# deeppowers/deeppowers

Hardware: AMD Instinct MI355X
Metric: ciphertext-mul/s (N=4096, 4 RNS limbs) (higher is better)
Workload: dtype u64

## Files before the change

deeppowers_amd/csrc/dpfhe_cabi.hip:

```cpp
#include <dlfcn.h>
#include <hip/hip_runtime.h>

#include <algorithm>
#include <atomic>
#include <cstdio>
#include <cstdlib>
#include <cstring>
#include <mutex>
#include <new>
#include <string>
#include <type_traits>
#include <vector>

#include "../../include/dpfhe.h"
#include "base_ext.h"
#include "compact.h"
#include "encode.h"
#include "expand.h"
#include "noise.h"
#include "plain_add.h"
#include "kernels_large.h"
#include "kernels_misc.h"
#include "launch.h"
#include "ntt_core.h"
// ... 1184 lines not shown
}

extern "C" int dpfhe_rescale_bsgs(dpfhe_ctx* c, uint64_t* d_out2, const uint64_t* d_in_qp, const uint64_t* d_addends, size_t n_add, size_t batch, void* stream) {
    const char* what = "dpfhe_rescale_bsgs";
    if (!c) return fail(DPFHE_INVALID_ARGUMENT, what, "null context");
    if (c->n_limbs < 2) return fail(DPFHE_INVALID_STATE, what, "no limb left to drop");
    if (batch == 0) return DPFHE_SUCCESS;
    if (!d_out2 || !d_in_qp || (n_add && !d_addends) || misaligned(d_out2) || misaligned(d_in_qp) || misaligned(d_addends))
        return fail(DPFHE_INVALID_ARGUMENT, what, "null or misaligned buffer");
    const size_t L = c->n_limbs, Ld = L - 1;
    const int n = 1 << c->log2n;
    const int chunks = (n + 511) / 512;
    if (overlaps(d_out2, batch * 2 * Ld * n, d_in_qp, batch * 2 * L * n) || (n_add && overlaps(d_out2, batch * 2 * Ld * n, d_addends, n_add * batch * 2 * Ld * n)))
        return fail(DPFHE_INVALID_ARGUMENT, what, "output overlaps an input");
    const size_t blocks = batch * 2 * Ld * (size_t)chunks;
    if (blocks > kMaxGrid) return fail(DPFHE_INVALID_ARGUMENT, what, "batch too large for one launch");
    DPFHE_ON_DEVICE(c, what);
    hipStream_t s = static_cast<hipStream_t>(stream);
    with_ctx_arith(c, [&](auto arith) {
        hipLaunchKernelGGL((rescale_bsgs_kernel<decltype(arith)>), dim3((unsigned)blocks), dim3(256), 0, s, d_out2, d_in_qp, d_addends, n_add, batch, c->lc, c->d_rescale, (int)L, n, chunks);
    });
    return check_launch("rescale_bsgs kernel launch");
}

extern "C" int dpfhe_apply_galois(dpfhe_ctx* c, uint64_t* d_out, const uint64_t* d_in, size_t n_rns_polys, uint32_t galois_elt, void* stream) {
    if (!c) return fail(DPFHE_INVALID_ARGUMENT, "dpfhe_apply_galois", "null context");
    const unsigned two_n = 2u << c->log2n;
    if (!(galois_elt & 1u) || galois_elt >= two_n) return fail(DPFHE_INVALID_ARGUMENT, "dpfhe_apply_galois", "galois_elt must be odd and < 2N");
    if (n_rns_polys == 0) return DPFHE_SUCCESS;
    if (!d_out || !d_in || misaligned(d_out) || misaligned(d_in) ||
        overlaps(d_out, n_rns_polys * ((size_t)c->n_limbs << c->log2n), d_in, n_rns_polys * ((size_t)c->n_limbs << c->log2n)))
        return fail(DPFHE_INVALID_ARGUMENT, "dpfhe_apply_galois", "null, misaligned or aliased buffer");
    const size_t npolys = n_rns_polys * c->n_limbs;
    if (npolys > kMaxGrid) return fail(DPFHE_INVALID_ARGUMENT, "dpfhe_apply_galois", "batch too large for one launch");
    DPFHE_ON_DEVICE(c, "dpfhe_apply_galois");
    const unsigned inv = galois_inverse(galois_elt, two_n);
    hipLaunchKernelGGL(galois_kernel, dim3((unsigned)npolys), dim3(256), 0, static_cast<hipStream_t>(stream), d_out, d_in, c->lc, (int)c->n_limbs,
                       1 << c->log2n, inv);
    return check_launch("galois kernel launch");
}

extern "C" int dpfhe_matvec_plain(dpfhe_ctx* c, uint64_t* d_y, const uint64_t* d_W, const uint64_t* d_x, size_t rows, size_t cols,
                                  void* stream) {
    if (!c) return fail(DPFHE_INVALID_ARGUMENT, "dpfhe_matvec_plain", "null context");
    if (rows == 0) return DPFHE_SUCCESS;
    if (cols == 0) return fail(DPFHE_INVALID_ARGUMENT, "dpfhe_matvec_plain", "cols must be > 0");
    if (!d_y || !d_W || !d_x || misaligned(d_y) || misaligned(d_W) || misaligned(d_x))
        return fail(DPFHE_INVALID_ARGUMENT, "dpfhe_matvec_plain", "null or misaligned buffer");
    const int n = 1 << c->log2n;
    constexpr int RT = 4;
    DPFHE_ON_DEVICE(c, "dpfhe_matvec_plain");
    hipStream_t s = static_cast<hipStream_t>(stream);
    if (c->fold) {
        constexpr int WPT = kMatvecWpt2;
        const int chunks = (n + 256 * WPT - 1) / (256 * WPT);
        const size_t slabs = c->n_limbs * (size_t)chunks, rtiles = (rows + RT - 1) / RT;
        const size_t blocks = ((slabs + 7) / 8) * 8 * rtiles;
        if (blocks > kMaxGrid) return fail(DPFHE_INVALID_ARGUMENT, "dpfhe_matvec_plain", "too many rows for one launch");
        const bool ntw = rows * cols * ((size_t)c->n_limbs << c->log2n) * sizeof(u64) > ((size_t)256 << 20);
        if (ntw) hipLaunchKernelGGL((matvec_fold_kernel<RT, 2, WPT, true>), dim3((unsigned)blocks), dim3(256), 0, s, d_y, d_W, d_x, c->lc, (int)c->n_limbs, n, chunks, rows,
                                    cols, (size_t)2, 1u, (unsigned)(rtiles * slabs));
        else hipLaunchKernelGGL((matvec_fold_kernel<RT, 2, WPT>), dim3((unsigned)blocks), dim3(256), 0, s, d_y, d_W, d_x, c->lc, (int)c->n_limbs, n, chunks, rows, cols,
                                (size_t)2, 1u, (unsigned)(rtiles * slabs));
        return check_launch("matvec kernel launch");
    }
    const int chunks = (n + 511) / 512;
    const size_t slabs = c->n_limbs * (size_t)chunks;
    const size_t blocks = ((slabs + 7) / 8) * 8 * ((rows + RT - 1) / RT);
    if (blocks > kMaxGrid) return fail(DPFHE_INVALID_ARGUMENT, "dpfhe_matvec_plain", "too many rows for one launch");
    hipLaunchKernelGGL((matvec_kernel<ShoupArith, RT>), dim3((unsigned)blocks), dim3(256), 0, s, d_y, d_W, d_x, c->lc, (int)c->n_limbs, n, chunks, rows, cols);
    return check_launch("matvec kernel launch");
}

template <bool FOLD, int RT, int C, int WPT = 2>
static int matvec_multi_launch(const dpfhe_ctx* c, const char* what, u64* ys, const u64* d_W, const u64* xs, size_t rows, size_t cols, size_t n_rhs, size_t groups,
                               hipStream_t s) {
    const int n = 1 << c->log2n, chunks = (n + 256 * WPT - 1) / (256 * WPT);
    const size_t slabs = c->n_limbs * (size_t)chunks, rtiles = (rows + RT - 1) / RT, tiles = rtiles * slabs;
    const size_t blocks = ((slabs + 7) / 8) * 8 * rtiles * groups;
    if (blocks > kMaxGrid) return fail(DPFHE_INVALID_ARGUMENT, what, "too many rows for one launch");
    if constexpr (!FOLD)
        hipLaunchKernelGGL((matvec_multi_kernel<ShoupArith, RT, C>), dim3((unsigned)blocks), dim3(256), 0, s, ys, d_W, xs, c->lc, (int)c->n_limbs, n, chunks, rows, cols,
                           n_rhs * 2, (unsigned)groups, (unsigned)tiles);
    else if (rows % RT == 0 && cols % FoldArith::kDot30Period == 0)
        hipLaunchKernelGGL((matvec_fold_kernel<RT, C, WPT, false, kMatvecWd, true>), dim3((unsigned)blocks), dim3(256), 0, s, ys, d_W, xs, c->lc, (int)c->n_limbs, n, chunks,
                           rows, cols, n_rhs * 2, (unsigned)groups, (unsigned)tiles);
    else
        hipLaunchKernelGGL((matvec_fold_kernel<RT, C, WPT, false, kMatvecWd>), dim3((unsigned)blocks), dim3(256), 0, s, ys, d_W, xs, c->lc, (int)c->n_limbs, n, chunks,
                           rows, cols, n_rhs * 2, (unsigned)groups, (unsigned)tiles);
    return check_launch("matvec_multi kernel launch");
}

extern "C" int dpfhe_matvec_plain_multi(dpfhe_ctx* c, uint64_t* d_y, const uint64_t* d_W, const uint64_t* d_x, size_t rows, size_t cols, size_t n_rhs,
                                        void* stream) {
    const char* what = "dpfhe_matvec_plain_multi";
    if (!c) return fail(DPFHE_INVALID_ARGUMENT, what, "null context");
    if (rows == 0 || n_rhs == 0) return DPFHE_SUCCESS;
    if (cols == 0) return fail(DPFHE_INVALID_ARGUMENT, what, "cols must be > 0");
    if (!d_y || !d_W || !d_x || misaligned(d_y) || misaligned(d_W) || misaligned(d_x)) return fail(DPFHE_INVALID_ARGUMENT, what, "null or misaligned buffer");
    if (n_rhs == 1) return dpfhe_matvec_plain(c, d_y, d_W, d_x, rows, cols, stream);
    const size_t poly = (size_t)c->n_limbs << c->log2n;
    hipStream_t s = static_cast<hipStream_t>(stream);
    DPFHE_ON_DEVICE(c, what);
    const size_t pairs = n_rhs / 2;
    const uint64_t* x_last = d_x + (n_rhs - 1) * 2 * poly;
    uint64_t* y_last = d_y + (n_rhs - 1) * 2 * poly;
    int rc = DPFHE_SUCCESS;
    if (c->fold) {
        if (pairs) rc = matvec_multi_launch<true, kMatvecRt4, 4, kMatvecWpt4>(c, what, d_y, d_W, d_x, rows, cols, n_rhs, pairs, s);
        if (!rc && (n_rhs & 1)) rc = matvec_multi_launch<true, 4, 2, kMatvecWpt2>(c, what, y_last, d_W, x_last, rows, cols, n_rhs, 1, s);
    } else {
        if (pairs) rc = matvec_multi_launch<false, 4, 4>(c, what, d_y, d_W, d_x, rows, cols, n_rhs, pairs, s);
        if (!rc && (n_rhs & 1)) rc = matvec_multi_launch<false, 4, 2>(c, what, y_last, d_W, x_last, rows, cols, n_rhs, 1, s);
    }
    return rc;
}

extern "C" int dpfhe_matvec_scalar(dpfhe_ctx* c, uint64_t* d_y, const uint64_t* d_w, const uint64_t* d_x, size_t rows, size_t cols,
                                   void* stream) {
    if (!c) return fail(DPFHE_INVALID_ARGUMENT, "dpfhe_matvec_scalar", "null context");
    if (rows == 0) return DPFHE_SUCCESS;
    if (cols == 0) return fail(DPFHE_INVALID_ARGUMENT, "dpfhe_matvec_scalar", "cols must be > 0");
    if (!d_y || !d_w || !d_x || misaligned(d_y) || misaligned(d_x) || (reinterpret_cast<uintptr_t>(d_w) & 7))
        return fail(DPFHE_INVALID_ARGUMENT, "dpfhe_matvec_scalar", "null or misaligned buffer");
    const int n = 1 << c->log2n;
    const int chunks = (n + 511) / 512;
    constexpr int RT = 8;
    const size_t blocks = ((rows + RT - 1) / RT) * c->n_limbs * (size_t)chunks;
    if (blocks > kMaxGrid) return fail(DPFHE_INVALID_ARGUMENT, "dpfhe_matvec_scalar", "too many rows for one launch");
    DPFHE_ON_DEVICE(c, "dpfhe_matvec_scalar");
    hipStream_t s = static_cast<hipStream_t>(stream);
    with_ctx_arith(c, [&](auto arith) {
        hipLaunchKernelGGL((matvec_scalar_kernel<decltype(arith), RT>), dim3((unsigned)blocks), dim3(256), 0, s, d_y, d_w, d_x, c->lc, (int)c->n_limbs, n, chunks, rows, cols);
    });
    return check_launch("matvec_scalar kernel launch");
}

extern "C" int dpfhe_reduce_sum(dpfhe_ctx* c, uint64_t* d_out, const uint64_t* d_in, size_t count, size_t components, void* stream) {
    if (!c) return fail(DPFHE_INVALID_ARGUMENT, "dpfhe_reduce_sum", "null context");
    if (components == 0 || count == 0) return fail(DPFHE_INVALID_ARGUMENT, "dpfhe_reduce_sum", "count and components must be > 0");
    if (!d_out || !d_in || misaligned(d_out) || misaligned(d_in)) return fail(DPFHE_INVALID_ARGUMENT, "dpfhe_reduce_sum", "null or misaligned buffer");
    const size_t blocks = components * c->n_limbs;
    if (blocks > kMaxGrid) return fail(DPFHE_INVALID_ARGUMENT, "dpfhe_reduce_sum", "too many components");
    DPFHE_ON_DEVICE(c, "dpfhe_reduce_sum");
    const int n = 1 << c->log2n;
    const int chunks = (n + 511) / 512;
    const size_t words_per_item = components * c->n_limbs * (size_t)n;
    const size_t want = count / 8 ? count / 8 : 1;
    const unsigned splits = (unsigned)(want < (size_t)kReduceSplits ? want : (size_t)kReduceSplits);
    hipStream_t s = static_cast<hipStream_t>(stream);
    if (blocks * (size_t)chunks * splits > kMaxGrid) return fail(DPFHE_INVALID_ARGUMENT, "dpfhe_reduce_sum", "too many components for one launch");
    HIP_TRY(hipMemsetAsync(d_out, 0, words_per_item * sizeof(u64), s));
    const unsigned poly_chunks = (unsigned)(blocks * chunks);
    unsigned grid = poly_chunks * splits;
    if (count > 512 && grid > 2u * (unsigned)c->n_cu) grid = 2u * (unsigned)c->n_cu;
    hipLaunchKernelGGL(reduce_partial_kernel, dim3(grid), dim3(256), 0, s, d_out, d_in, c->lc, (int)c->n_limbs, n, chunks, count, words_per_item,
                       poly_chunks, splits);
    if (int e = check_launch("reduce_sum partial kernel launch")) return e;
    hipLaunchKernelGGL(reduce_final_kernel, dim3((unsigned)(blocks * chunks)), dim3(256), 0, s, d_out, c->lc, (int)c->n_limbs, n, chunks);
    return check_launch("reduce_sum kernel launch");
}

extern "C" int dpfhe_canonicalize_sum(dpfhe_ctx* c, uint64_t* d_io, size_t n_rns_polys, void* stream) {
    if (!c) return fail(DPFHE_INVALID_ARGUMENT, "dpfhe_canonicalize_sum", "null context");
    if (n_rns_polys == 0) return DPFHE_SUCCESS;
    if (!d_io || misaligned(d_io)) return fail(DPFHE_INVALID_ARGUMENT, "dpfhe_canonicalize_sum", "null or misaligned buffer");
    const int n = 1 << c->log2n, chunks = (n + 511) / 512;
    const size_t blocks = n_rns_polys * c->n_limbs * (size_t)chunks;
    if (blocks > kMaxGrid) return fail(DPFHE_INVALID_ARGUMENT, "dpfhe_canonicalize_sum", "batch too large for one launch");
    DPFHE_ON_DEVICE(c, "dpfhe_canonicalize_sum");
    hipLaunchKernelGGL(reduce_final_kernel, dim3((unsigned)blocks), dim3(256), 0, static_cast<hipStream_t>(stream), d_io, c->lc, (int)c->n_limbs, n, chunks);
    return check_launch("canonicalize_sum kernel launch");
}

static int base_extend_common(dpfhe_ctx* c, int mode, uint64_t* d_out, size_t out_stride_limbs, const uint64_t* d_in, size_t in_stride_limbs, uint32_t src0, uint32_t ns,
                              uint32_t dst0, uint32_t nd, uint64_t multiplier, size_t n_polys, void* stream, const char* what) {
    if (!c) return fail(DPFHE_INVALID_ARGUMENT, what, "null context");
    if (n_polys == 0) return DPFHE_SUCCESS;
    const uint32_t L = c->n_limbs;
    if (ns == 0 || ns > (uint32_t)kBxMaxSrc || nd == 0 || nd > (uint32_t)kBxMaxDst || src0 > L || ns > L - src0 || dst0 > L || nd > L - dst0)
        return fail(DPFHE_INVALID_ARGUMENT, what, "1..10 source limbs and 1..20 destination limbs inside the context");
    if (mode == 1 && !(dst0 >= src0 + ns || dst0 + nd <= src0)) return fail(DPFHE_INVALID_ARGUMENT, what, "the dropped limbs and the kept limbs must be disjoint");
    if (!d_out || !d_in || misaligned(d_out) || misaligned(d_in) || out_stride_limbs < nd || in_stride_limbs < ns) return fail(DPFHE_INVALID_ARGUMENT, what, "null or misaligned buffer, or an item stride shorter than its limbs");
    const size_t n = (size_t)1 << c->log2n;
    const int chunks = (int)((n + 511) / 512);
    if (n_polys * (size_t)chunks > kMaxGrid) return fail(DPFHE_INVALID_ARGUMENT, what, "batch too large for one launch");
    {
        const uint64_t* in_lo = mode == 1 ? d_in - (size_t)src0 * n : d_in;
        const size_t in_words = mode == 1 ? n_polys * (size_t)L * n : ((n_polys - 1) * in_stride_limbs + ns) * n;
        if (overlaps(d_out, ((n_polys - 1) * out_stride_limbs + nd) * n, in_lo, in_words)) return fail(DPFHE_INVALID_ARGUMENT, what, "output overlaps the input");
    }
    const std::vector<uint64_t>& q = c->moduli;
    BaseExtArgs a{};
    a.n_src = (int)ns; a.n_dst = (int)nd;
    for (uint32_t i = 0; i < ns; ++i) a.src_limb[i] = (int)(src0 + i);
    for (uint32_t j = 0; j < nd; ++j) a.dst_limb[j] = (int)(dst0 + j);
    for (uint32_t i = 0; i < ns; ++i)
        for (uint32_t k = i + 1; k < ns; ++k) {
            if (q[src0 + i] == q[src0 + k]) return fail(DPFHE_INVALID_ARGUMENT, what, "source limbs must be distinct primes");
            a.inv[i][k] = h_powmod(q[src0 + i] % q[src0 + k], q[src0 + k] - 2, q[src0 + k]);
        }
    {
        unsigned __int128 carry = 0;
        for (int k = (int)ns - 1; k >= 0; --k) {
            const unsigned __int128 cur = carry * q[src0 + k] + (q[src0 + k] - 1);
            a.half[k] = (uint64_t)(cur / 2);
            carry = cur & 1;
        }
    }
    for (uint32_t j = 0; j < nd; ++j) {
        const uint64_t pj = q[dst0 + j];
        uint64_t Qm = 1;
        for (uint32_t i = 0; i < ns; ++i) { a.q_mod[i][j] = q[src0 + i] % pj; Qm = h_mulmod(Qm, a.q_mod[i][j], pj); }
        a.Q_mod[j] = Qm;
        if (mode == 1) {
            if (Qm == 0) return fail(DPFHE_INVALID_ARGUMENT, what, "a kept limb divides the dropped modulus");
            a.Q_inv[j] = h_powmod(Qm, pj - 2, pj);
            a.mul_dst[j] = multiplier % pj;
        }
    }
    for (uint32_t i = 0; i < ns; ++i) a.mul_src[i] = multiplier % q[src0 + i];
    DPFHE_ON_DEVICE(c, what);
    hipStream_t s = static_cast<hipStream_t>(stream);
    const unsigned grid = (unsigned)(n_polys * (size_t)chunks);
    const size_t in_dst_off = mode == 1 ? ((size_t)dst0 - (size_t)src0) * n : 0;
    const int rc = with_ctx_arith(c, [&](auto arith) {
        return launch_base_extend<decltype(arith)>(mode, d_out, out_stride_limbs * n, d_in, in_stride_limbs * n, in_dst_off, a, c->lc, (int)n, chunks, grid, s);
    });
    if (rc) return fail(DPFHE_INVALID_STATE, what, "no kernel for this number of source limbs");
    return check_launch("base_extend kernel launch");
}
extern "C" int dpfhe_base_extend(dpfhe_ctx* c, uint64_t* d_out, size_t out_stride_limbs, const uint64_t* d_in, size_t in_stride_limbs, uint32_t src_limb0, uint32_t n_src,
                                 uint32_t dst_limb0, uint32_t n_dst, size_t n_polys, void* stream) {
    return base_extend_common(c, 0, d_out, out_stride_limbs, d_in, in_stride_limbs, src_limb0, n_src, dst_limb0, n_dst, 1, n_polys, stream, "dpfhe_base_extend");
}
extern "C" int dpfhe_scale_round(dpfhe_ctx* c, uint64_t* d_out, size_t out_stride_limbs, const uint64_t* d_in, uint32_t drop_limb0, uint32_t n_drop, uint32_t keep_limb0,
                                 uint32_t n_keep, uint64_t multiplier, size_t n_polys, void* stream) {
    if (!c) return fail(DPFHE_INVALID_ARGUMENT, "dpfhe_scale_round", "null context");
    if (multiplier == 0) return fail(DPFHE_INVALID_ARGUMENT, "dpfhe_scale_round", "multiplier must be > 0");
    const size_t n = (size_t)1 << c->log2n;
    return base_extend_common(c, 1, d_out, out_stride_limbs, d_in ? d_in + (size_t)drop_limb0 * n : nullptr, c->n_limbs, drop_limb0, n_drop, keep_limb0, n_keep, multiplier, n_polys, stream,
                              "dpfhe_scale_round");
}

extern "C" int dpfhe_copy(dpfhe_ctx* c, uint64_t* d_dst, const uint64_t* d_src, size_t n_words, void* stream) {
    if (!c) return fail(DPFHE_INVALID_ARGUMENT, "dpfhe_copy", "null context");
    if (n_words == 0) return DPFHE_SUCCESS;
    if (!d_dst || !d_src || misaligned(d_dst) || misaligned(d_src) || (n_words & 1)) return fail(DPFHE_INVALID_ARGUMENT, "dpfhe_copy", "null or misaligned buffer, or an odd word count");
    if (overlaps(d_dst, n_words, d_src, n_words)) return fail(DPFHE_INVALID_ARGUMENT, "dpfhe_copy", "buffers overlap");
    const size_t n_vec = n_words / 2, blocks = (n_vec + 2047) / 2048;
    if (blocks > kMaxGrid) return fail(DPFHE_INVALID_ARGUMENT, "dpfhe_copy", "too many words for one launch");
    DPFHE_ON_DEVICE(c, "dpfhe_copy");
    if (n_words * 16 > (size_t)256 << 20)
        hipLaunchKernelGGL(copy_kernel<true>, dim3((unsigned)blocks), dim3(256), 0, static_cast<hipStream_t>(stream), reinterpret_cast<U64x2*>(d_dst),
                           reinterpret_cast<const U64x2*>(d_src), n_vec);
    else
        hipLaunchKernelGGL(copy_kernel<false>, dim3((unsigned)blocks), dim3(256), 0, static_cast<hipStream_t>(stream), reinterpret_cast<U64x2*>(d_dst),
                           reinterpret_cast<const U64x2*>(d_src), n_vec);
    return check_launch("copy kernel launch");
}

static int expand_args(const char* what, const void* buf, size_t components, uint32_t component, const uint8_t* seed, uint64_t first_item, size_t batch,
                       ExpandKey& key) {
    if (!buf || !seed) return fail(DPFHE_INVALID_ARGUMENT, what, "null buffer or seed");
    if (component >= components) return fail(DPFHE_INVALID_ARGUMENT, what, "component must be < components");
    if (first_item > ((uint64_t)1 << 32) || batch > ((uint64_t)1 << 32) - first_item) return fail(DPFHE_INVALID_ARGUMENT, what, "first_item + batch must be <= 2^32");
    std::memcpy(key.w, seed, 32);
    return DPFHE_SUCCESS;
}

static int check_host_ring(const char* what, const uint64_t* moduli, uint32_t n_limbs, uint32_t log2_n) {
    if (n_limbs == 0 || log2_n < 8 || log2_n > (uint32_t)kMaxLog2N) return fail(DPFHE_INVALID_ARGUMENT, what, "n_limbs >= 1 and log2_n in [8, 16]");
    for (uint32_t l = 0; l < n_limbs; ++l)
        if (moduli[l] < 3 || (moduli[l] >> 60) || !(moduli[l] & 1)) return fail(DPFHE_INVALID_ARGUMENT, what, "moduli must be odd, >= 3 and < 2^60");
    return DPFHE_SUCCESS;
}

extern "C" int dpfhe_expand_uniform(dpfhe_ctx* c, uint64_t* d_buf, size_t batch, size_t components, uint32_t component, const uint8_t seed[32],
                                    uint64_t first_item, void* stream) {
    if (!c) return fail(DPFHE_INVALID_ARGUMENT, "dpfhe_expand_uniform", "null context");
    ExpandKey key;
    if (int rc = expand_args("dpfhe_expand_uniform", d_buf, components, component, seed, first_item, batch, key)) return rc;
    if (misaligned(d_buf)) return fail(DPFHE_INVALID_ARGUMENT, "dpfhe_expand_uniform", "misaligned buffer");
    if (batch == 0) return DPFHE_SUCCESS;
    DPFHE_ON_DEVICE(c, "dpfhe_expand_uniform");
    if (launch_expand_uniform((int)c->log2n, d_buf, batch, components, component, c->n_limbs, c->lc, key, (uint32_t)first_item, static_cast<hipStream_t>(stream)))
        return fail(DPFHE_INVALID_ARGUMENT, "dpfhe_expand_uniform", "batch too large for one launch");
    return check_launch("expand_uniform kernel launch");
}

extern "C" int dpfhe_expand_uniform_host(const uint64_t* moduli, uint32_t n_limbs, uint32_t log2_n, uint64_t* out, size_t batch, size_t components,
                                         uint32_t component, const uint8_t seed[32], uint64_t first_item) {
    if (!moduli) return fail(DPFHE_INVALID_ARGUMENT, "dpfhe_expand_uniform_host", "null moduli");
    ExpandKey key;
    if (int rc = expand_args("dpfhe_expand_uniform_host", out, components, component, seed, first_item, batch, key)) return rc;
    if (int rc = check_host_ring("dpfhe_expand_uniform_host", moduli, n_limbs, log2_n)) return rc;
    expand_uniform_host((int)log2_n, moduli, n_limbs, out, batch, components, component, key, (uint32_t)first_item);
    return DPFHE_SUCCESS;
}

static bool inverse_mod(uint64_t t, uint64_t q, uint64_t& inv) {
    int64_t r0 = (int64_t)q, r1 = (int64_t)(t % q), s0 = 0, s1 = 1;
    while (r1) {
        const int64_t k = r0 / r1, r2 = r0 - k * r1, s2 = s0 - k * s1;
        r0 = r1; r1 = r2; s0 = s1; s1 = s2;
    }
    if (r0 != 1) return false;
    inv = s0 < 0 ? (uint64_t)(s0 + (int64_t)q) : (uint64_t)s0;
    return true;
}
// ... 462 lines not shown
```

deeppowers_amd/csrc/kernels_misc.h:

```cpp
#pragma once
#include <hip/hip_runtime.h>

#include "launch.h"
#include "modarith.h"

namespace dpfhe {

enum DyOp { DY_MUL = 0, DY_MUL_ADD = 1, DY_ADD = 2, DY_SUB = 3, DY_NEG = 4 };

template <class Arith, int OP>
__device__ __forceinline__ u64 dy_apply(u64 a, u64 b, u64 acc, const LimbConst& lc) {
    if (OP == DY_MUL) return Arith::mul_var(a, b, lc);
    if (OP == DY_MUL_ADD) return add_mod(acc, Arith::mul_var(a, b, lc), lc.q);
    if (OP == DY_ADD) return add_mod(a, b, lc.q);
    if (OP == DY_SUB) return sub_mod(a, b, lc.q);
    return neg_mod(a, lc.q);
}

template <bool NT>
__device__ __forceinline__ U64x2 ld_vec(const U64x2* p) {
    if (NT) { U64x2 v; v.a = __builtin_nontemporal_load(&p->a); v.b = __builtin_nontemporal_load(&p->b); return v; }
    return *p;
}
template <bool NT>
__device__ __forceinline__ void st_vec(U64x2* p, const U64x2& v) {
    if (NT) { __builtin_nontemporal_store(v.a, &p->a); __builtin_nontemporal_store(v.b, &p->b); }
    else *p = v;
}

template <class Arith, int OP, bool NT = false>
__global__ __launch_bounds__(256) void dyadic_kernel(u64* out, const u64* a, const u64* b, const LimbConst* lcs, int n_limbs, int n, int b_period = 0) {
    const size_t p = blockIdx.x;
    const LimbConst lc = lcs[p % (size_t)n_limbs];
    const U64x2* pa = reinterpret_cast<const U64x2*>(a + p * n);
    const U64x2* pb = reinterpret_cast<const U64x2*>(b + (b_period ? p % (size_t)b_period : p) * n);
    U64x2* po = reinterpret_cast<U64x2*>(out + p * n);
    const int nv = n >> 1;
    constexpr int UN = 4;
    for (int base = threadIdx.x; base < nv; base += 256 * UN) {
        U64x2 va[UN], vb[UN], vc[UN];
#pragma unroll
        for (int u = 0; u < UN; ++u) {
            const int i = base + u * 256;
            if (i < nv) {
                va[u] = ld_vec<NT>(pa + i);
                if (OP != DY_NEG) vb[u] = b_period ? pb[i] : ld_vec<NT>(pb + i);
                if (OP == DY_MUL_ADD) vc[u] = ld_vec<NT>(po + i);
            }
        }
#pragma unroll
        for (int u = 0; u < UN; ++u) {
            const int i = base + u * 256;
            if (i < nv) {
                U64x2 r;
                r.a = dy_apply<Arith, OP>(va[u].a, vb[u].a, vc[u].a, lc);
                r.b = dy_apply<Arith, OP>(va[u].b, vb[u].b, vc[u].b, lc);
                st_vec<NT>(po + i, r);
            }
        }
    }
}

template <bool NT>
__global__ __launch_bounds__(256) void copy_kernel(U64x2* __restrict__ dst, const U64x2* __restrict__ src, size_t n_vec) {
    const size_t base = (size_t)blockIdx.x * 2048 + threadIdx.x;
    if ((size_t)blockIdx.x * 2048 + 2048 <= n_vec) {
        U64x2 v[8];
#pragma unroll
        for (int u = 0; u < 8; ++u) {
            if (NT) { v[u].a = __builtin_nontemporal_load(&src[base + u * 256].a); v[u].b = __builtin_nontemporal_load(&src[base + u * 256].b); }
            else v[u] = src[base + u * 256];
        }
#pragma unroll
        for (int u = 0; u < 8; ++u) {
            if (NT) { __builtin_nontemporal_store(v[u].a, &dst[base + u * 256].a); __builtin_nontemporal_store(v[u].b, &dst[base + u * 256].b); }
            else dst[base + u * 256] = v[u];
        }
    } else {
        for (size_t i = base; i < n_vec; i += 256) dst[i] = src[i];
    }
}

constexpr int kReduceSplits = 15;

__global__ __launch_bounds__(256) void reduce_partial_kernel(u64* out, const u64* in, const LimbConst* lcs, int n_limbs, int n, int chunks,
                                                             size_t count, size_t words_per_item, unsigned poly_chunks, unsigned nsplit) {
    for (unsigned work = blockIdx.x; work < poly_chunks * nsplit; work += gridDim.x) {
        const unsigned pc = work % poly_chunks;
        const size_t split = work / poly_chunks;
        const size_t p = pc / (unsigned)chunks;
        const int w = (int)(pc % (unsigned)chunks) * 512 + threadIdx.x * 2;
        if (w >= n) continue;
        const u64 q = lcs[p % (size_t)n_limbs].q;
        const size_t lo = count * split / nsplit, hi = count * (split + 1) / nsplit;
        const u64* src = in + p * n + w;
        u64 s0 = 0, s1 = 0;
        size_t it = lo;
        for (; it + 4 <= hi; it += 4) {
            U64x2 v[4];
#pragma unroll
            for (int u = 0; u < 4; ++u) {
                v[u] = *reinterpret_cast<const U64x2*>(src + (it + u) * words_per_item);
            }
#pragma unroll
            for (int u = 0; u < 4; ++u) { s0 = csub(s0 + v[u].a, q); s1 = csub(s1 + v[u].b, q); }
        }
        for (; it < hi; ++it) {
            const U64x2 v = *reinterpret_cast<const U64x2*>(src + it * words_per_item);
            s0 = csub(s0 + v.a, q); s1 = csub(s1 + v.b, q);
        }
        if (hi > lo) {
            atomicAdd(reinterpret_cast<unsigned long long*>(out + p * n + w), (unsigned long long)s0);
            atomicAdd(reinterpret_cast<unsigned long long*>(out + p * n + w + 1), (unsigned long long)s1);
        }
    }
}

__global__ __launch_bounds__(256) void reduce_final_kernel(u64* out, const LimbConst* lcs, int n_limbs, int n, int chunks) {
    const size_t p = blockIdx.x / chunks;
    const int w = (int)(blockIdx.x % chunks) * 512 + threadIdx.x * 2;
    if (w >= n) return;
    const u64 q = lcs[p % (size_t)n_limbs].q;
    U64x2* o = reinterpret_cast<U64x2*>(out + p * n + w);
    U64x2 v = *o;
    v.a = csub(csub(csub(csub(v.a, 8 * q), 4 * q), 2 * q), q);
    v.b = csub(csub(csub(csub(v.b, 8 * q), 4 * q), 2 * q), q);
    *o = v;
}

struct Acc128 {
    u64 lo, hi;
};
__device__ __forceinline__ void acc_mac(Acc128& acc, u64 a, u64 b) {
    const u64 lo = a * b, hi = mulhi64(a, b);
    acc.lo += lo;
    acc.hi += hi + (acc.lo < lo);
}
template <class Arith>
__device__ __forceinline__ u64 acc_reduce(const Acc128& acc, const LimbConst& lc, u64 two64_mod_q) {
    if (Arith::kFold) {
        const u64 h = FoldArith::mul60_full(acc.hi, two64_mod_q, (u32)lc.d);
        const u64 l = FoldArith::reduce(acc.lo, lc);
        return FoldArith::canon(h + l, lc);
    } else {
        const u64 h = ShoupArith::mul_var(acc.hi % lc.q, two64_mod_q, lc);
        return add_mod(h, acc.lo % lc.q, lc.q);
    }
}

template <class Arith, int RT>
__global__ __launch_bounds__(256) void matvec_kernel(u64* y, const u64* W, const u64* x, const LimbConst* lcs, int n_limbs, int n,
                                                     int chunks, size_t rows, size_t cols) {
    const size_t L = (size_t)n_limbs;
    const unsigned n_slabs = (unsigned)L * (unsigned)chunks, R = (unsigned)((rows + RT - 1) / RT);
    const unsigned id = blockIdx.x, q = id >> 3, slab = (q / R) * 8u + (id & 7u);
    if (slab >= n_slabs) return;
    const int chunk = (int)(slab % chunks);
    const int limb = (int)(slab / chunks);
    const size_t row0 = (size_t)(q % R) * RT;
    const int w0 = chunk * 512 + threadIdx.x * 2;
    if (w0 >= n) return;
    const LimbConst lc = lcs[limb];
    const u64 two64 = lc.two64;
    const size_t wstride = L * n, xstride = 2 * L * n, rstride = cols * L * n;
    Acc128 acc[RT][2][2];
#pragma unroll
    for (int r = 0; r < RT; ++r)
#pragma unroll
        for (int c = 0; c < 2; ++c) acc[r][c][0] = acc[r][c][1] = Acc128{0, 0};
    const u64* wp = W + (row0 * cols * L + limb) * n + w0;
    const u64* xp = x + (size_t)limb * n + w0;
    size_t since = 0;
    U64x2 x0 = *reinterpret_cast<const U64x2*>(xp), x1 = *reinterpret_cast<const U64x2*>(xp + L * n), w[RT];
#pragma unroll
    for (int r = 0; r < RT; ++r) w[r] = (row0 + r < rows) ? *reinterpret_cast<const U64x2*>(wp + r * rstride) : U64x2{0, 0};
    for (size_t j = 0; j < cols; ++j) {
        if (j > 0) {
            x0 = *reinterpret_cast<const U64x2*>(xp + j * xstride);
            x1 = *reinterpret_cast<const U64x2*>(xp + j * xstride + L * n);
#pragma unroll
            for (int r = 0; r < RT; ++r) w[r] = (row0 + r < rows) ? *reinterpret_cast<const U64x2*>(wp + r * rstride + j * wstride) : U64x2{0, 0};
        }
#pragma unroll
        for (int r = 0; r < RT; ++r) {
            acc_mac(acc[r][0][0], w[r].a, x0.a); acc_mac(acc[r][0][1], w[r].b, x0.b);
            acc_mac(acc[r][1][0], w[r].a, x1.a); acc_mac(acc[r][1][1], w[r].b, x1.b);
        }
        if (++since == 128) {
#pragma unroll
            for (int r = 0; r < RT; ++r)
#pragma unroll
                for (int c = 0; c < 2; ++c)
#pragma unroll
                    for (int k = 0; k < 2; ++k) acc[r][c][k] = Acc128{acc_reduce<Arith>(acc[r][c][k], lc, two64), 0};
            since = 0;
        }
    }
#pragma unroll
    for (int r = 0; r < RT; ++r) {
        if (row0 + r >= rows) break;
        u64* yp = y + (((row0 + r) * 2) * L + limb) * n + w0;
        *reinterpret_cast<U64x2*>(yp) = U64x2{acc_reduce<Arith>(acc[r][0][0], lc, two64), acc_reduce<Arith>(acc[r][0][1], lc, two64)};
        *reinterpret_cast<U64x2*>(yp + L * n) = U64x2{acc_reduce<Arith>(acc[r][1][0], lc, two64), acc_reduce<Arith>(acc[r][1][1], lc, two64)};
    }
}

template <class Arith, int RT, int C>
__global__ __launch_bounds__(256) void matvec_multi_kernel(u64* y, const u64* W, const u64* x, const LimbConst* lcs, int n_limbs, int n,
                                                           int chunks, size_t rows, size_t cols, size_t polys_per_col ,
                                                           unsigned n_groups, unsigned n_tiles) {
    const size_t L = (size_t)n_limbs;
    const unsigned n_slabs = (unsigned)L * (unsigned)chunks, R = n_tiles / n_slabs;
    const unsigned id = blockIdx.x, lane = id & 7u, q = id >> 3;
    const unsigned group = q % n_groups, rt = (q / n_groups) % R, slab = (q / (n_groups * R)) * 8u + lane;
    if (slab >= n_slabs) return;
    const int chunk = (int)(slab % chunks);
    const int limb = (int)(slab / chunks);
    const size_t row0 = (size_t)rt * RT;
    const int w0 = chunk * 512 + threadIdx.x * 2;
    if (w0 >= n) return;
    x += (size_t)group * C * L * n;
    y += (size_t)group * C * L * n;
    const LimbConst lc = lcs[limb];
    const u64 two64 = lc.two64;
    const size_t wstride = L * n, xstride = polys_per_col * L * n, rstride = cols * L * n;
    Acc128 acc[RT][C][2];
#pragma unroll
    for (int r = 0; r < RT; ++r)
#pragma unroll
        for (int c = 0; c < C; ++c) acc[r][c][0] = acc[r][c][1] = Acc128{0, 0};
    const u64* wp = W + (row0 * cols * L + limb) * n + w0;
    const u64* xp = x + (size_t)limb * n + w0;
    size_t since = 0;
    U64x2 w[RT], xv[C];
#pragma unroll
    for (int r = 0; r < RT; ++r) w[r] = (row0 + r < rows) ? *reinterpret_cast<const U64x2*>(wp + r * rstride) : U64x2{0, 0};
#pragma unroll
    for (int c = 0; c < C; ++c) xv[c] = *reinterpret_cast<const U64x2*>(xp + (size_t)c * L * n);
    for (size_t j = 0; j < cols; ++j) {
        const size_t jn = j + 1 < cols ? j + 1 : j;
        U64x2 wn[RT], xn[C];
#pragma unroll
        for (int r = 0; r < RT; ++r) wn[r] = (row0 + r < rows) ? *reinterpret_cast<const U64x2*>(wp + r * rstride + jn * wstride) : U64x2{0, 0};
#pragma unroll
        for (int c = 0; c < C; ++c) xn[c] = *reinterpret_cast<const U64x2*>(xp + jn * xstride + (size_t)c * L * n);
#pragma unroll
        for (int c = 0; c < C; ++c) {
#pragma unroll
            for (int r = 0; r < RT; ++r) { acc_mac(acc[r][c][0], w[r].a, xv[c].a); acc_mac(acc[r][c][1], w[r].b, xv[c].b); }
        }
#pragma unroll
        for (int r = 0; r < RT; ++r) w[r] = wn[r];
#pragma unroll
        for (int c = 0; c < C; ++c) xv[c] = xn[c];
        if (++since == 128) {
#pragma unroll
            for (int r = 0; r < RT; ++r)
#pragma unroll
                for (int c = 0; c < C; ++c)
#pragma unroll
                    for (int k = 0; k < 2; ++k) acc[r][c][k] = Acc128{acc_reduce<Arith>(acc[r][c][k], lc, two64), 0};
            since = 0;
        }
    }
#pragma unroll
    for (int r = 0; r < RT; ++r) {
        if (row0 + r >= rows) break;
// ... 634 lines not shown
```

Baseline: 2.380 million.

## Add thin reduce-sum kernel with lazy accumulation and buffer loads

Adds a reduce_thin_kernel used when folding is enabled and the item count is large. It keeps a rotating register pipeline of in-flight loads, accumulates without per-add modular reduction and folds every ten terms, issues raw buffer loads, and loops over a grid of at most one block per CU. This is meant to cut the per-element conditional-subtract cost and the launch oversubscription of the old reduction. In exchange it relies on sums staying below 2^64 and on the fold arithmetic being correct.

Result: faster. 2.425 million, median of 6 (+1.9%).

```diff
diff --git a/deeppowers_amd/csrc/dpfhe_cabi.hip b/deeppowers_amd/csrc/dpfhe_cabi.hip
--- a/deeppowers_amd/csrc/dpfhe_cabi.hip
+++ b/deeppowers_amd/csrc/dpfhe_cabi.hip
@@ -1360,10 +1360,20 @@
     if (blocks * (size_t)chunks * splits > kMaxGrid) return fail(DPFHE_INVALID_ARGUMENT, "dpfhe_reduce_sum", "too many components for one launch");
     HIP_TRY(hipMemsetAsync(d_out, 0, words_per_item * sizeof(u64), s));
     const unsigned poly_chunks = (unsigned)(blocks * chunks);
-    unsigned grid = poly_chunks * splits;
-    if (count > 512 && grid > 2u * (unsigned)c->n_cu) grid = 2u * (unsigned)c->n_cu;
-    hipLaunchKernelGGL(reduce_partial_kernel, dim3(grid), dim3(256), 0, s, d_out, d_in, c->lc, (int)c->n_limbs, n, chunks, count, words_per_item,
-                       poly_chunks, splits);
+    const unsigned items = poly_chunks * splits;
+    if (c->fold && count > 512) {
+        const unsigned grid = items < (unsigned)c->n_cu ? items : (unsigned)c->n_cu;
+        const unsigned threads = n / 2 < 256 ? (unsigned)n / 2 : 256u;
+        unsigned log2_chunks = 0;
+        while ((1 << log2_chunks) < chunks) ++log2_chunks;
+        hipLaunchKernelGGL(reduce_thin_kernel, dim3(grid), dim3(threads), 0, s, d_out, d_in, c->lc, (unsigned)c->n_limbs, (unsigned)n, log2_chunks,
+                           count / splits, (unsigned)(count % splits), words_per_item, poly_chunks, splits);
+    } else {
+        unsigned grid = items;
+        if (count > 512 && grid > 2u * (unsigned)c->n_cu) grid = 2u * (unsigned)c->n_cu;
+        hipLaunchKernelGGL(reduce_partial_kernel, dim3(grid), dim3(256), 0, s, d_out, d_in, c->lc, (int)c->n_limbs, n, chunks, count, words_per_item,
+                           poly_chunks, splits);
+    }
     if (int e = check_launch("reduce_sum partial kernel launch")) return e;
     hipLaunchKernelGGL(reduce_final_kernel, dim3((unsigned)(blocks * chunks)), dim3(256), 0, s, d_out, c->lc, (int)c->n_limbs, n, chunks);
     return check_launch("reduce_sum kernel launch");
diff --git a/deeppowers_amd/csrc/kernels_misc.h b/deeppowers_amd/csrc/kernels_misc.h
--- a/deeppowers_amd/csrc/kernels_misc.h
+++ b/deeppowers_amd/csrc/kernels_misc.h
@@ -3,6 +3,7 @@
 
 #include "launch.h"
 #include "modarith.h"
+#include "reduce_thin.h"
 
 namespace dpfhe {
 
@@ -113,6 +114,32 @@
             atomicAdd(reinterpret_cast<unsigned long long*>(out + p * n + w), (unsigned long long)s0);
             atomicAdd(reinterpret_cast<unsigned long long*>(out + p * n + w + 1), (unsigned long long)s1);
         }
+    }
+}
+
+__global__ __launch_bounds__(256) void reduce_thin_kernel(u64* __restrict__ out, const u64* __restrict__ in, const LimbConst* __restrict__ lcs, unsigned n_limbs,
+                                                          unsigned n, unsigned log2_chunks, size_t per, unsigned rem, size_t words_per_item, unsigned poly_chunks,
+                                                          unsigned nsplit) {
+    const unsigned lane = threadIdx.x * 16u;
+    unsigned pc = blockIdx.x % poly_chunks, split = blockIdx.x / poly_chunks;
+    while (split < nsplit) {
+        const unsigned p = pc >> log2_chunks, w0 = (pc & ((1u << log2_chunks) - 1u)) * 512u;
+        const LimbConst lc = lcs[p % n_limbs];
+        const size_t lo = split * per + (split < rem ? split : rem), hi = (split + 1) * per + (split + 1 < rem ? split + 1 : rem);
+        const u64* src = in + (size_t)p * n + w0;
+        const U64x2 sum = thin_sum([&](size_t it) {
+            typedef unsigned v4u __attribute__((ext_vector_type(4)));
+            const __amdgpu_buffer_rsrc_t rs = __builtin_amdgcn_make_buffer_rsrc(const_cast<u64*>(src + it * words_per_item), 0, 0x7fffffff, 0x00020000);
+            const v4u t = __builtin_amdgcn_raw_buffer_load_b128(rs, (int)lane, 0, 0);
+            return U64x2{((u64)t.y << 32) | t.x, ((u64)t.w << 32) | t.z};
+        }, lo, hi, lc);
+        if (hi > lo) {
+            u64* o = reinterpret_cast<u64*>(reinterpret_cast<char*>(out + (size_t)p * n + w0) + lane);
+            atomicAdd(reinterpret_cast<unsigned long long*>(o), (unsigned long long)sum.a);
+            atomicAdd(reinterpret_cast<unsigned long long*>(o + 1), (unsigned long long)sum.b);
+        }
+        pc += gridDim.x;
+        while (pc >= poly_chunks) { pc -= poly_chunks; ++split; }
     }
 }
 
diff --git a/deeppowers_amd/csrc/reduce_thin.h b/deeppowers_amd/csrc/reduce_thin.h
--- /dev/null
+++ b/deeppowers_amd/csrc/reduce_thin.h
@@ -0,0 +1,62 @@
+#pragma once
+#include <stddef.h>
+
+#include "modarith.h"
+
+namespace dpfhe {
+
+constexpr int kThinDepth = 5;
+constexpr int kThinRounds = 2;
+static_assert(kThinDepth * kThinRounds <= 14, "a folded word plus the terms of one pass must stay below 2^64");
+
+DPF_HD void thin_keep_order(u64& s0, u64& s1) {
+#if defined(__HIP_DEVICE_COMPILE__)
+    asm volatile("" : "+v"(s0), "+v"(s1) : : "memory");
+#else
+    (void)s0; (void)s1;
+#endif
+}
+
+DPF_HD void thin_add(u64& s, u64 x) {
+    DPFHE_EMU_ASSERT(s + x >= s);
+    s += x;
+}
+
+template <class Load>
+DPF_HD U64x2 thin_sum(Load ld, size_t lo, size_t hi, const LimbConst& lc) {
+    u64 s0 = 0, s1 = 0;
+    size_t it = lo;
+    if (it + kThinDepth <= hi) {
+        U64x2 v[kThinDepth];
+#pragma unroll
+        for (int u = 0; u < kThinDepth; ++u) v[u] = ld(it + u);
+        it += kThinDepth;
+        for (; it + kThinRounds * kThinDepth <= hi; it += kThinRounds * kThinDepth) {
+#pragma unroll
+            for (int u = 0; u < kThinRounds * kThinDepth; ++u) {
+                thin_add(s0, v[u % kThinDepth].a); thin_add(s1, v[u % kThinDepth].b);
+                thin_keep_order(s0, s1);
+                v[u % kThinDepth] = ld(it + u);
+            }
+            s0 = FoldArith::reduce(s0, lc); s1 = FoldArith::reduce(s1, lc);
+        }
+        for (; it + kThinDepth <= hi; it += kThinDepth) {
+#pragma unroll
+            for (int u = 0; u < kThinDepth; ++u) {
+                thin_add(s0, v[u].a); thin_add(s1, v[u].b);
+                thin_keep_order(s0, s1);
+                v[u] = ld(it + u);
+            }
+        }
+#pragma unroll
+        for (int u = 0; u < kThinDepth; ++u) { thin_add(s0, v[u].a); thin_add(s1, v[u].b); }
+        s0 = FoldArith::reduce(s0, lc); s1 = FoldArith::reduce(s1, lc);
+    }
+    for (; it < hi; ++it) {
+        const U64x2 v = ld(it);
+        thin_add(s0, v.a); thin_add(s1, v.b);
+    }
+    return U64x2{FoldArith::canon(s0, lc), FoldArith::canon(s1, lc)};
+}
+
+}
```
